# edwinb-ai/MolecularDynamics.jl

Hardware: AMD Instinct MI355X
Metric: particle-steps/sec + achieved HBM GB/s, 1M LJ particles rho=0.897, 1/2/4/8 GPUs (higher is better)
Workload: dtype f64; 1 GPU; BASELINE configs[2]: N=1048576 monodisperse LJ 3D rho=0.897 r_cut=2.5 dt=0.001 NVT Bussi tau=0.1 kT=1.4737, per GPU; particles_per_gpu=1048576, parallelism=1 GPU, step_loop=fused (k_step_tile: one launch per step + k_finalize), global_particles=1048576, tiled_force_kernel=True, max_tile_halo=2081, energies_every_step=False, thermo_frequency=2589

## Files before the change

### include/mdhip.h

```cpp
#ifndef MDHIP_H
#define MDHIP_H

#include <stdint.h>

#ifdef __cplusplus
extern "C" {
#endif

typedef struct md_ctx md_ctx;

enum { MD_POT_LJ = 0, MD_POT_PSEUDOHS = 1, MD_POT_POLYDISPERSE = 2, MD_POT_LJ_MODIFIED = 3, MD_POT_CUSTOM = 100 };

enum { MD_NVE = 0, MD_NVT = 1 };

int md_create(int dim, int64_t n_particles, const double *box, double list_cutoff, int device_id, md_ctx **out);
int md_destroy(md_ctx *ctx);

const char *md_last_error(md_ctx *ctx);

int md_set_potential(md_ctx *ctx, int kind, const double *params, int nparams);

int md_set_potential_source(md_ctx *ctx, const char *hip_src, const char *entry_name, const double *params,
                            int nparams);

// ... 41 lines not shown

int md_stress_setup(md_ctx *ctx, int nlags);
int md_stress_sample(md_ctx *ctx);
int md_stress_tensor(md_ctx *ctx, double *kin, double *vir);
int md_stress_read(md_ctx *ctx, int64_t *nsamples, double *sum_kin, double *sum_vir, int64_t *ncorr, double *corr);
int md_stress_reset(md_ctx *ctx);

int md_kinetic(md_ctx *ctx, double *kinetic);

int md_scale_velocities(md_ctx *ctx, double s);

typedef struct {
    int64_t steps;
    int64_t rebuilds;
    int64_t violations;
    int64_t n_ghost;
    int64_t max_neighbors;
    double avg_neighbors;
    int64_t force_launches;
    double force_ms;
    int64_t max_halo;
    int64_t tiled;
    int64_t prunes;
    int64_t kickdrift_launches;
    double kickdrift_ms;
    int64_t fused;
    int64_t walked_outer;
    int64_t walked_inner;
    int64_t prune_launches_timed;
    double prune_ms;
    int64_t rebuilds_timed;
    double rebuild_ms;
    int64_t fused_build;
} md_stats;
int md_profile(md_ctx *ctx, int enable);
int md_get_stats(md_ctx *ctx, md_stats *out);

int md_create_domain(int dim, int64_t n_global, int64_t n_cap, const double *box, double list_cutoff,
                     int device_id, int rank, int nranks, md_ctx **out);
int md_dom_set_uniform(md_ctx *ctx, int uniform, double sigma);
int md_dom_upload(md_ctx *ctx, int64_t n_own, const int32_t *ids, const double *x, const double *v, const double *f,
                  const int32_t *images, const double *diameters);
int md_dom_download(md_ctx *ctx, int64_t cap, int64_t *n_own, int32_t *ids, double *x, double *v, double *f,
                    int32_t *images);
int md_dom_migrate_pack(md_ctx *ctx, int64_t *nsend );
int md_dom_migrate_unpack(md_ctx *ctx, const int64_t *nrecv );
int md_dom_halo_pack(md_ctx *ctx, int64_t *nsend );
int md_dom_halo_unpack(md_ctx *ctx, const int64_t *nrecv );
int md_dom_build(md_ctx *ctx);
int md_dom_set_step_buffers(md_ctx *ctx, void *send_left, void *send_right, void *recv_left, void *recv_right,
                            int64_t capacity_doubles);
int md_dom_get_sendbuf(md_ctx *ctx, int side, int64_t ndoubles, void *dst, int dst_is_device);
int md_dom_put_recvbuf(md_ctx *ctx, int side, int64_t ndoubles, const void *src, int src_is_device);
int md_dom_step_begin(md_ctx *ctx, double dt, int *violated);
int md_dom_step_end(md_ctx *ctx, double dt, int want_uw, double *uwk);
int md_dom_forces(md_ctx *ctx, double dt, int kick, int want_uw, double *uwk);
int md_dom_set_scale(md_ctx *ctx, double scale);
int md_dom_counts(md_ctx *ctx, int64_t *out );

int md_set_stream(md_ctx *ctx, void *hip_stream);
int md_dom_async_begin(md_ctx *ctx, int64_t nsteps, double dt, int ensemble, double tau, double nf, const double *ktemp,
                       const double *r1, const double *r2, int64_t prune_interval, void *flag_dev ,
                       void *kuw_dev );
int md_dom_step_a(md_ctx *ctx, double dt, int step);
int md_dom_step_b(md_ctx *ctx, double dt, int step, int want_uw);
int md_dom_step_c(md_ctx *ctx, int step, int want_uw);
// ... 19 lines not shown
```

### moleculardynamics/jl_amd/_lib.py

```python
import ctypes as C
import os

_HERE = os.path.dirname(os.path.abspath(__file__))
SO_PATH = os.path.join(_HERE, "csrc", "libmdhip.so")

MD_POT_LJ, MD_POT_PSEUDOHS, MD_POT_POLYDISPERSE, MD_POT_LJ_MODIFIED, MD_POT_CUSTOM = 0, 1, 2, 3, 100
MD_NVE, MD_NVT = 0, 1

EXPORTS = [
    "md_create", "md_destroy", "md_last_error", "md_set_potential", "md_set_potential_source", "md_set_skin",
    "md_set_inner_skin",
    "md_upload", "md_download", "md_snapshot_begin", "md_snapshot_end", "md_compute_forces", "md_neighbor_pairs", "md_run", "md_kinetic",
    "md_scale_velocities", "md_profile", "md_get_stats", "md_version", "md_fire_minimize", "md_run_brownian",
    "md_create_domain", "md_dom_set_uniform", "md_dom_upload", "md_dom_download", "md_dom_migrate_pack",
    "md_dom_migrate_unpack", "md_dom_halo_pack", "md_dom_halo_unpack", "md_dom_build", "md_dom_get_sendbuf",
    "md_dom_put_recvbuf", "md_dom_set_step_buffers", "md_dom_step_begin", "md_dom_step_end", "md_dom_forces", "md_dom_set_scale",
    "md_dom_counts", "md_set_stream", "md_dom_async_begin", "md_dom_step_a", "md_dom_step_b", "md_dom_step_c",
    "md_dom_async_end", "md_dom_comm_unique_id", "md_dom_comm_init", "md_dom_run_window", "md_dom_rebuild",
    "md_dom_enable_pruning", "md_dom_max_disp0", "md_dom_invalidate_inner",
    "md_rdf_setup", "md_rdf_sample", "md_rdf_read", "md_rdf_reset",
    "md_dyn_setup", "md_dyn_origin", "md_dyn_sample", "md_dyn_read", "md_dyn_reset",
    "md_sq_setup", "md_sq_sample", "md_sq_rho", "md_sq_read", "md_sq_reset",
    "md_stress_setup", "md_stress_sample", "md_stress_tensor", "md_stress_read", "md_stress_reset",
]


class MdStats(C.Structure):
    _fields_ = [("steps", C.c_int64), ("rebuilds", C.c_int64), ("violations", C.c_int64), ("n_ghost", C.c_int64),
                ("max_neighbors", C.c_int64), ("avg_neighbors", C.c_double), ("force_launches", C.c_int64),
                ("force_ms", C.c_double), ("max_halo", C.c_int64), ("tiled", C.c_int64), ("prunes", C.c_int64),
                ("kickdrift_launches", C.c_int64), ("kickdrift_ms", C.c_double), ("fused", C.c_int64),
                ("walked_outer", C.c_int64), ("walked_inner", C.c_int64), ("prune_launches_timed", C.c_int64),
                ("prune_ms", C.c_double), ("rebuilds_timed", C.c_int64), ("rebuild_ms", C.c_double),
                ("fused_build", C.c_int64)]


class MdhipError(RuntimeError):
    pass


_lib = None


def load():
    global _lib
    if _lib is not None:
        return _lib
    if not os.path.exists(SO_PATH):
        raise MdhipError(
            f"{SO_PATH} not found: build it with `python -c 'import __graft_entry__ as g; g.build()'` or "
            "`make -C moleculardynamics/jl_amd/csrc`. There is no CPU fallback.")
    L = C.CDLL(SO_PATH)
    vp, dp, ip = C.c_void_p, C.POINTER(C.c_double), C.POINTER(C.c_int32)
    L.md_create.argtypes = [C.c_int, C.c_int64, dp, C.c_double, C.c_int, C.POINTER(vp)]
    L.md_create.restype = C.c_int
    L.md_destroy.argtypes = [vp]
    L.md_destroy.restype = C.c_int
    L.md_last_error.argtypes = [vp]
    L.md_last_error.restype = C.c_char_p
    L.md_set_potential.argtypes = [vp, C.c_int, dp, C.c_int]
    L.md_set_potential.restype = C.c_int
    L.md_set_potential_source.argtypes = [vp, C.c_char_p, C.c_char_p, dp, C.c_int]
    L.md_set_potential_source.restype = C.c_int
    L.md_set_skin.argtypes = [vp, C.c_double]
    L.md_set_skin.restype = C.c_int
    L.md_set_inner_skin.argtypes = [vp, C.c_double]
    L.md_set_inner_skin.restype = C.c_int
# ... 107 lines not shown
```

### moleculardynamics/jl_amd/csrc/md_kernels.hpp

```cpp
#ifndef MD_RTC
#pragma once
#include <hip/hip_runtime.h>
#include <stdint.h>
#else
typedef __hip_internal::uint64_t uint64_t;
typedef __hip_internal::uint32_t uint32_t;
typedef __hip_internal::int32_t int32_t;
typedef __hip_internal::uint16_t uint16_t;
#endif

#define MD_BLOCK 256
#define MD_WAVE 64
#define MD_SENTINEL_POS 1.0e100
#define MD_VAL_SRC_BITS 26
#define MD_VAL_SRC_MASK ((1u << MD_VAL_SRC_BITS) - 1u)
#define MD_NO_VIOLATION 0x7fffffff

enum { POT_LJ = 0, POT_PSEUDOHS = 1, POT_POLYDISPERSE = 2, POT_LJ_MOD = 3, POT_CUSTOM = 100 };

struct DevState {
    double4 *pos;
    double *v[3];
    double *f[3];
    int32_t *img[3];
// ... 823 lines not shown
        uint32_t j = row[(size_t)r * 64];
        uint32_t loc;
        if (j == sentinel) {
            loc = (uint32_t)H;
        } else {
            uint32_t h = (j * 2654435761u) >> (32 - MD_HT_BITS);
            while (keys[h] != j) h = (h + 1) & (MD_HT - 1);
            loc = vals[h];
        }
        row16[row_off(r, lane)] = (uint16_t)(loc * (uint32_t)rs);
    }
}

#ifndef MD_RTC
#include "md_build_tile.hpp"
#endif

struct PruneRow {
    unsigned char *base;
    unsigned off;
};
__device__ __forceinline__ void prune_append(unsigned entry, PruneRow &pr, unsigned long long &acc, int &cin)
{
    unsigned lo = (unsigned)acc, hi = (unsigned)(acc >> 32);
    lo = __builtin_amdgcn_alignbit(hi, lo, 16);
    hi = __builtin_amdgcn_alignbit(entry, hi, 16);
    acc = ((unsigned long long)hi << 32) | lo;
    ++cin;
    if ((cin & 3) == 0) {
        *(unsigned long long *)(pr.base + pr.off) = acc;
        pr.off += 512u;
    }
}

template <int D, int POT, bool UNIFORM, bool WANT_UW, bool PRUNE, int NQ>
__device__ __forceinline__ void tile_pair_block(const unsigned char *smem, const unsigned (&o)[NQ], const double4 &pi,
                                                const PotParams &pp, PruneRow &rin64, double rin2,
                                                unsigned long long &acc, int &cin, double &fx, double &fy, double &fz,
                                                double &us, double &ws, const uint16_t *remap8)
{
    double xj[NQ], yj[NQ], zj[NQ], wj[NQ];
#pragma unroll
    for (int q = 0; q < NQ; ++q) {
        typedef const volatile __attribute__((address_space(3))) double lds_cvd;
        if constexpr (!UNIFORM && D == 3) {
            typedef double md_d2 __attribute__((ext_vector_type(2)));
            typedef const __attribute__((address_space(3))) md_d2 lds_d2;
            lds_d2 *r2 = (lds_d2 *)(smem + o[q]);
            md_d2 a = r2[0], b = r2[1];
            xj[q] = a.x;
            yj[q] = a.y;
            zj[q] = b.x;
            wj[q] = b.y;
        } else {
            lds_cvd *rec = (lds_cvd *)(smem + o[q]);
            xj[q] = rec[0];
            yj[q] = rec[1];
            if constexpr (D == 3) zj[q] = rec[2];
            if constexpr (!UNIFORM) wj[q] = rec[3];
        }
    }
    if constexpr (POT == POT_LJ && UNIFORM && !WANT_UW && D == 3) {
        double dxq[NQ], dyq[NQ], dzq[NQ], dm[NQ];
        unsigned tmin = 0xffffffffu;
        double d2k[PRUNE ? NQ : 1];
#pragma unroll
        for (int q = 0; q < NQ; ++q) {
            dxq[q] = xj[q] - pi.x;
            dyq[q] = yj[q] - pi.y;
            dzq[q] = zj[q] - pi.z;
            double d2 = dxq[q] * dxq[q];
            d2 = __builtin_fma(dyq[q], dyq[q], d2);
            d2 = __builtin_fma(dzq[q], dzq[q], d2);
            if constexpr (PRUNE) d2k[q] = d2;
            int hi = __double2hiint(d2);
            unsigned t = (unsigned)hi - pp.c2_k;
            tmin = min(tmin, t);
            hi = ((int)t < 0) ? hi : 0x5fe00000;
            dm[q] = __hiloint2double(hi, __double2loint(d2));
        }
        if constexpr (PRUNE) {
#pragma unroll
            for (int q = 0; q < NQ; ++q) asm volatile("" : "+v"(d2k[q]));
#pragma unroll
            for (int q = 0; q < NQ; ++q)
                if (d2k[q] <= rin2)
                    prune_append(remap8 ? (unsigned)remap8[o[q] >> 3] : o[q], rin64, acc, cin);
        }
        if (__any(tmin <= 2u)) {
#pragma unroll
            for (int q = 0; q < NQ; ++q) {
                double d2 = dxq[q] * dxq[q];
                d2 = __builtin_fma(dyq[q], dyq[q], d2);
                d2 = __builtin_fma(dzq[q], dzq[q], d2);
                unsigned t = (unsigned)__double2hiint(d2) - pp.c2_k;
                if (t <= 2u) {
                    bool hit = d2_ref<3>(dxq[q], dyq[q], dzq[q]) < pp.c2;
                    dm[q] = __hiloint2double(hit ? __double2hiint(d2) : 0x5fe00000, __double2loint(d2));
                }
            }
        }
#pragma unroll
        for (int q = 0; q < NQ; q += 2) {
            double ip = md_rcp1(dm[q] * dm[q + 1]);
            double z[2] = {dm[q + 1] * ip, dm[q] * ip};
#pragma unroll
            for (int h = 0; h < 2; ++h) {
                double z2 = z[h] * z[h];
                double t = __builtin_fma(pp.ljA, z2 * z[h], -pp.ljB);
                double fpr = (z2 * z2) * t;
                fx = __builtin_fma(-fpr, dxq[q + h], fx);
                fy = __builtin_fma(-fpr, dyq[q + h], fy);
                fz = __builtin_fma(-fpr, dzq[q + h], fz);
            }
        }
    } else
#pragma unroll
    for (int q = 0; q < NQ; ++q) {
        double dx = xj[q] - pi.x;
        double dy = yj[q] - pi.y;
        double dz = 0.0;
        if constexpr (D == 3) dz = zj[q] - pi.z;
        double d2 = d2_ref<D>(dx, dy, dz);
        if constexpr (PRUNE) {
            if (d2 <= rin2)
                prune_append(remap8 ? (unsigned)remap8[o[q] >> 3] : o[q], rin64, acc, cin);
        }
        bool hit = d2 < pp.c2;
        double d2m = mask_d2(d2, hit);
        double u = 0.0, fpr;
        pair_eval<POT, UNIFORM, WANT_UW>(d2m, pi.w, UNIFORM ? 0.0 : wj[q], pp, u, fpr);
        fx = __builtin_fma(-fpr, dx, fx);
        fy = __builtin_fma(-fpr, dy, fy);
        if constexpr (D == 3) fz = __builtin_fma(-fpr, dz, fz);
        if constexpr (WANT_UW) {
            us += u;
            ws = __builtin_fma(fpr, hit ? d2 : 0.0, ws);
        }
    }
}

template <int D, int POT, bool UNIFORM, bool WANT_UW, bool PRUNE>
__device__ __forceinline__ void tile_pair_loop(const unsigned char *smem, const ushort4 *row4,
                                               ushort4 (&jn)[MD_UNROLL / 4], int m_lane, int H,
                                               const double4 &pi, const PotParams &pp, PruneRow &rin64,
                                               double rin2, unsigned long long &acc, int &cin, double &fx, double &fy,
                                               double &fz, double &us, double &ws, const uint16_t *remap8 = nullptr)
{
    constexpr int G = MD_UNROLL / 4;
    static_assert(G == 2, "the tail handling below assumes two groups per iteration");
    (void)H;
    const int m = __builtin_amdgcn_readfirstlane(m_lane);
    int r = 0;
    for (; r + MD_UNROLL <= m; r += MD_UNROLL) {
        unsigned o[MD_UNROLL];
#pragma unroll
        for (int g = 0; g < G; ++g) {
            o[4 * g + 0] = jn[g].x;
            o[4 * g + 1] = jn[g].y;
            o[4 * g + 2] = jn[g].z;
            o[4 * g + 3] = jn[g].w;
        }
#pragma unroll
        for (int g = 0; g < G; ++g) {
            int rg = r + MD_UNROLL + 4 * g;
            jn[g] = row4[(size_t)(((rg < m) ? rg : 0) >> 2) * 64];
        }
        tile_pair_block<D, POT, UNIFORM, WANT_UW, PRUNE, MD_UNROLL>(smem, o, pi, pp, rin64, rin2, acc, cin, fx, fy, fz, us,
                                                                     ws, remap8);
    }
    if (r < m) {
        unsigned o[4] = {jn[0].x, jn[0].y, jn[0].z, jn[0].w};
        tile_pair_block<D, POT, UNIFORM, WANT_UW, PRUNE, 4>(smem, o, pi, pp, rin64, rin2, acc, cin, fx, fy, fz, us, ws,
                                                            remap8);
    }
}

template <int D, bool UNIFORM>
__device__ __forceinline__ void tile_prune_tail(DevState &s, Scalars *sc, int H , int k, bool active, int lane, int wt,
                                                const double4 &pi, PruneRow rin64, int32_t *nmax_in,
                                                unsigned long long acc, int cin)
{
    constexpr int RS = UNIFORM ? 24 : 32;
    {
        const unsigned long long sent = (unsigned long long)(H * RS);
        const unsigned long long sent4 = sent | (sent << 16) | (sent << 32) | (sent << 48);
        int mw = wave_max_i((cin + 3) & ~3);
        int g = cin >> 2;
        if (cin & 3) {
            int p = cin & 3;
            *(unsigned long long *)(rin64.base + rin64.off) = (acc >> (16 * (4 - p))) | (sent4 << (16 * p));
            rin64.off += 512u;
            ++g;
        }
        for (; g < (mw >> 2); ++g, rin64.off += 512u) *(unsigned long long *)(rin64.base + rin64.off) = sent4;
        if (lane == 0) nmax_in[wt] = mw;
        double dd = 0.0;
        if (active) {
#pragma unroll
            for (int c = 0; c < D; ++c) {
                double xc = pos_get(pi, c);
                s.x1[c][k] = xc;
                double d = xc - s.x0[c][k];
                dd = __builtin_fma(d, d, dd);
            }
        }
        double wm = wave_max_d(dd);
// ... 193 lines not shown
                s.v[2][k] = vz;
                ke += vz * vz;
            }
        }
    } else {
        us = 0.0;
        ws = 0.0;
    }
    if constexpr (KICK) {
        double t = block_sum(ke, red);
        if (threadIdx.x == 0) partials[bid] = t;
    }
    if constexpr (WANT_UW) {
        double tu = block_sum(us, red);
        double tw = block_sum(ws, red);
        if (threadIdx.x == 0) {
            partials[nblk_total + bid] = tu;
            partials[2 * nblk_total + bid] = tw;
        }
    }
    MD_SSTAMP(5);
#undef MD_SSTAMP
}

struct StepBufs {
    const double2 *recA;
    double2 *recB;
    size_t rstride;
    const double *fA[3];
    double *fB[3];
    double4 *posB;
};

template <int D, int POT, bool UNIFORM, bool WANT_UW, bool PRUNE>
__global__ void __launch_bounds__(MD_TILE)
    k_step_tile(int n, DevState s, StepBufs sb, PotParams pp, const uint16_t *__restrict__ nlist16, int maxn,
                const int32_t *__restrict__ nmax_tile, const uint32_t *__restrict__ halo, int hcap,
                const int32_t *__restrict__ halo_count, double dt, double skin_half, double inner_half, int use_d1,
                double *__restrict__ partials, int nblk_total, Scalars *__restrict__ sc, int step,
                uint16_t *__restrict__ rows_in, int32_t *__restrict__ nmax_in, double rin2,
                long long *__restrict__ stamps, uint32_t *__restrict__ halo_in, int hcap_in,
                int32_t *__restrict__ halo_in_count, const int32_t *__restrict__ tile_list = nullptr)
{
#define MD_SSTAMP(i)                                                                                   \
    do {                                                                                               \
        if (stamps && (threadIdx.x & 63) == 0)                                                         \
            stamps[((size_t)blockIdx.x * 4 + (threadIdx.x >> 6)) * 8 + (i)] = (long long)clock64();   \
    } while (0)
    constexpr int RS = UNIFORM ? 24 : 32;
    extern __shared__ __attribute__((aligned(16))) unsigned char smem[];
    __shared__ double red[16];
    if (sc->first_viol < step) return;
    MD_SSTAMP(0);
    int bid = xcd_remap(blockIdx.x, gridDim.x);
    if (tile_list) bid = tile_list[bid];
    int H = halo_count[bid];
    const uint32_t *hl = halo + (size_t)bid * hcap;
    int k = bid * MD_TILE + threadIdx.x;
    bool active = k < n;
    int kk = active ? k : n - 1;
    int lane = threadIdx.x & 63;
    int wt = bid * (MD_TILE / 64) + (threadIdx.x >> 6);
    const ushort4 *row4 = (const ushort4 *)(nlist16 + ((size_t)wt * maxn) * 64) + lane;
    PruneRow rin64;
    rin64.base = PRUNE ? (unsigned char *)(rows_in + ((size_t)__builtin_amdgcn_readfirstlane(wt) * maxn) * 64) : nullptr;
    rin64.off = (unsigned)lane * 8u;
    unsigned long long acc = 0ull;
    int cin = 0;
    int m = nmax_tile[wt];
    const double alpha = sc->scale;
    const double adt = alpha * dt;
    const double2 *RA0 = sb.recA, *RA1 = RA0 + sb.rstride, *RA2 = RA1 + sb.rstride, *RA3 = RA2 + sb.rstride;
    double2 a0 = RA0[kk], a1 = RA1[kk], a2 = RA2[kk];
    double sig_own = pp.sig_u;
    if constexpr (!UNIFORM) sig_own = RA3[kk].x;
    double fprev[3] = {0.0, 0.0, 0.0}, xr[3] = {0.0, 0.0, 0.0};
#pragma unroll
    for (int c = 0; c < D; ++c) {
        fprev[c] = sb.fA[c][kk];
        xr[c] = PRUNE ? s.x0[c][kk] : s.x1[c][kk];
    }
    constexpr int G = MD_UNROLL / 4;
    ushort4 jn[G];
#pragma unroll
    for (int g = 0; g < G; ++g) jn[g] = row4[(size_t)((4 * g < m) ? g : 0) * 64];
    MD_SSTAMP(1);
#ifndef MD_STAGE_NB
#define MD_STAGE_NB ((!PRUNE && UNIFORM && !WANT_UW) ? 6 : 8)
#endif
    constexpr int NB = MD_STAGE_NB;
    for (int h0 = 0; h0 <= H; h0 += NB * MD_TILE) {
        uint32_t idx[NB];
#pragma unroll
        for (int i = 0; i < NB; ++i) {
            int h = h0 + i * MD_TILE + threadIdx.x;
            idx[i] = (h < H) ? hl[h] : 0xffffffffu;
        }
        double2 r0[NB], r1[NB], r2[NB], r3[NB];
#pragma unroll
        for (int i = 0; i < NB; ++i) {
            bool ok = idx[i] != 0xffffffffu;
            size_t j = ok ? (size_t)(idx[i] & 0x3ffffffu) : 0;
            r0[i] = RA0[j];
            r1[i] = RA1[j];
            r2[i] = RA2[j];
            if constexpr (!UNIFORM) r3[i] = RA3[j];
        }
#pragma unroll
        for (int i = 0; i < NB; ++i) {
            int h = h0 + i * MD_TILE + threadIdx.x;
            bool ok = idx[i] != 0xffffffffu;
            double x = __builtin_fma(adt, r1[i].y, r0[i].x);
            double y = __builtin_fma(adt, r2[i].x, r0[i].y);
            double z = (D == 3) ? __builtin_fma(adt, r2[i].y, r1[i].x) : 0.0;
            uint32_t code = ok ? (idx[i] >> 26) : 0u;
            if (code) shift_xyz(x, y, z, code, s.boxL, s.tric, s.cellA);
            if (!ok) {
                x = MD_SENTINEL_POS;
                y = MD_SENTINEL_POS;
                z = (D == 3) ? MD_SENTINEL_POS : 0.0;
            }
            if (h <= H) {
                double *rec = (double *)(smem + (size_t)h * RS);
                rec[0] = x;
                rec[1] = y;
                rec[2] = z;
                if constexpr (!UNIFORM) rec[3] = ok ? r3[i].x : 1.0;
            }
        }
    }
    const double pown[3] = {a0.x, a0.y, a1.x}, vown[3] = {a1.y, a2.x, a2.y};
    double vh[3] = {0.0, 0.0, 0.0}, xn[3] = {0.0, 0.0, 0.0};
    double disp2 = 0.0;
#pragma unroll
    for (int c = 0; c < D; ++c) {
        vh[c] = alpha * vown[c] + (fprev[c] * dt) / 2.0;
        xn[c] = __builtin_fma(adt, vown[c], pown[c]);
        double d = xn[c] - xr[c];
        disp2 = __builtin_fma(d, d, disp2);
    }
    const double4 pi = make_double4(xn[0], xn[1], xn[2], sig_own);
    if (active) sb.posB[k] = pi;
    {
        double d1 = use_d1 ? sqrt(__longlong_as_double((long long)sc->d1max2_bits)) : 0.0;
        double thr = fmin(inner_half, skin_half - d1);
        double thr2 = thr > 0.0 ? thr * thr : -1.0;
        if (__any(active && disp2 > thr2)) {
            if (lane == 0) atomicMin(&sc->first_viol, step);
        }
    }
    MD_SSTAMP(2);
    __syncthreads();
    MD_SSTAMP(3);
    double fx = 0.0, fy = 0.0, fz = 0.0, us = 0.0, ws = 0.0;
    tile_pair_loop<D, POT, UNIFORM, WANT_UW, PRUNE>(smem, row4, jn, m, H, pi, pp, rin64, rin2, acc, cin, fx, fy, fz, us, ws, nullptr);
    MD_SSTAMP(4);
    if constexpr (PRUNE) tile_prune_tail<D, UNIFORM>(s, sc, H, k, active, lane, wt, pi, rin64, nmax_in, acc, cin);
    double ke = 0.0;
    if (active) {
        const double fn[3] = {fx, fy, fz};
        const double h2 = (dt * dt) / 2.0;
        double vp[3] = {0.0, 0.0, 0.0}, pn[3] = {0.0, 0.0, 0.0};
#pragma unroll
        for (int c = 0; c < D; ++c) {
            sb.fB[c][k] = fn[c];
            vp[c] = vh[c] + (fn[c] * dt) / 2.0;
            pn[c] = __builtin_fma(h2, fn[c], xn[c]);
            ke += vp[c] * vp[c];
        }
        double2 *RB = sb.recB;
        RB[k] = make_double2(pn[0], pn[1]);
        RB[sb.rstride + k] = make_double2(pn[2], vp[0]);
        RB[2 * sb.rstride + k] = make_double2(vp[1], vp[2]);
        if constexpr (!UNIFORM) RB[3 * sb.rstride + k] = make_double2(sig_own, 0.0);
    } else {
        us = 0.0;
        ws = 0.0;
    }
    {
        double t = block_sum(ke, red);
        if (threadIdx.x == 0) partials[bid] = t;
    }
    if constexpr (WANT_UW) {
        double tu = block_sum(us, red);
        double tw = block_sum(ws, red);
        if (threadIdx.x == 0) {
            partials[nblk_total + bid] = tu;
            partials[2 * nblk_total + bid] = tw;
        }
    }
// ... 468 lines not shown
```

### moleculardynamics/jl_amd/csrc/mdhip.hip

```cpp
#include <cstring>
#include <cstdlib>
#include <unistd.h>

#include "md_kernels.hpp"
#include "md_domain.hpp"
#include "md_rdf.hpp"
#include "md_dyn.hpp"
#include "md_sq.hpp"
#include "md_stress.hpp"

#include <rocprim/rocprim.hpp>

#include <algorithm>
#include <climits>
#include <cmath>
#include <cstdio>
#include <cstring>
#include <stdexcept>
#include <string>
#include <vector>

#include "../../../include/mdhip.h"
#include "md_rtc.hpp"
#include "md_rccl.hpp"
// ... 157 lines not shown
    DBuf<Scalars> scal;
    DBuf<double> d_kt, d_r1, d_r2;

    DBuf<double> io_x, io_v, io_f, io_d;
    DBuf<int32_t> io_i;
    DBuf<double> snap_x;
    DBuf<int32_t> snap_i;
    double *pin_x = nullptr;
    int32_t *pin_i = nullptr;
    size_t pin_n = 0;
    hipStream_t copy_stream = nullptr;
    hipEvent_t ev_snap_ready = nullptr, ev_snap_copied = nullptr;
    bool snap_pending = false;

    bool list_valid = false;
    int64_t steps_since_build = 0;
    int64_t target_interval = 8;
    double inner_skin_req = 0.16;
    double inner_skin = 0.0;
    bool virtual_ghosts = false;
    bool inner_valid = false;
    bool prune_on = false;
    DBuf<double> x1[3];
    DBuf<uint16_t> nlist16_in;
    DBuf<int32_t> nmax_tile_in;
    int64_t steps_since_prune = 0;
    DBuf<double2> rec[2];
    DBuf<uint32_t> halo_in;
    DBuf<int32_t> halo_in_count;
    int hcap_in = 0;
    size_t tile_lds_in = 0;
    bool allow_inner_halo = true;
    bool inner_halo_live = false;
    int fz_a = 0;
    bool allow_fused = true;
    double d1_rate = 0.0;
    bool rate_known = false;
    double safety = 0.97;
    int64_t st_prunes = 0;

    int64_t st_steps = 0, st_rebuilds = 0, st_viol = 0;
    bool prof = false;
    int prof_stride = 1;
    int64_t prof_seen[2] = {0, 0};
    bool prof_open = false;
    std::vector<std::pair<hipEvent_t, hipEvent_t>> prof_ev;
    size_t prof_used = 0;
    double prof_ms_acc = 0.0;
    int64_t prof_launch_acc = 0;
    std::vector<int> prof_tag;
    double prof_kd_ms_acc = 0.0;
    int64_t prof_kd_launch_acc = 0;
    int64_t prof_prune_acc = 0;
    double prof_prune_ms_acc = 0.0;
    double prof_rebuild_ms_acc = 0.0;
    int64_t prof_rebuild_acc = 0;
    bool prof_cur_prune = false;
    bool last_run_fused = false;
    struct StepPart {
        const int32_t *list = nullptr;
        int count = 0;
        hipStream_t stream = nullptr;
        bool last = true;
    } part;

    struct Rdf {
// ... 478 lines not shown
    if (getenv("MDHIP_ROWSTATS")) {
        std::vector<int32_t> nn((size_t)n), nm((size_t)c->ntiles);
        HIPCHK(hipMemcpyAsync(nn.data(), c->nneigh.p, sizeof(int32_t) * n, hipMemcpyDeviceToHost, st));
        HIPCHK(hipMemcpyAsync(nm.data(), c->nmax_tile.p, sizeof(int32_t) * c->ntiles, hipMemcpyDeviceToHost, st));
        HIPCHK(hipStreamSynchronize(st));
        double mean = 0, padded = 0, sorted_p = 0, p8 = 0, s8 = 0;
        for (int i = 0; i < n; ++i) mean += nn[i];
        for (int w = 0; w < (n + 63) / 64; ++w) { padded += nm[w]; p8 += (nm[w] + 7) & ~7; }
        for (int t0 = 0; t0 + 256 <= n; t0 += 256) {
            std::vector<int> v(nn.begin() + t0, nn.begin() + t0 + 256);
            std::sort(v.begin(), v.end());
            for (int w = 0; w < 4; ++w) { int mx = (v[64 * w + 63] + 3) & ~3; sorted_p += mx; s8 += (mx + 7) & ~7; }
        }
        int nw = (n + 63) / 64;
        fprintf(stderr, "[mdhip] rows: mean %.2f  wave-max(4) %.2f  wave-max(8) %.2f  sorted-within-tile(4) %.2f  (8) %.2f\n",
                mean / n, padded / nw, p8 / nw, sorted_p / nw, s8 / nw);
    }
    c->list_valid = true;
    c->steps_since_build = 0;
    c->st_rebuilds++;
    c->inner_valid = false;
    c->prune_on = c->use_tiles && (!c->dom.on || c->dom.prune_enabled) && c->skin > 0.0 && c->inner_skin_req > 0.0 &&
                  c->inner_skin_req < 0.9 * c->skin && c->pot_kind != POT_CUSTOM;
    if (c->prune_on) {
        c->inner_skin = c->inner_skin_req;
        for (int d = 0; d < c->dim; ++d) c->x1[d].ensure(c->ncap);
        c->nlist16_in.ensure((size_t)c->ntiles * c->maxn * 64);
        c->nmax_tile_in.ensure(c->ntiles);
        const size_t target = (c->tile_rs == 24) ? (40 * 1024 - 256) : (53 * 1024);
        int cap_in = (int)std::min<size_t>((size_t)c->hstride, target / c->tile_rs - 1);
        if (c->dom.on || getenv("MDHIP_INNER_CAP_OUTER")) cap_in = c->hstride;
        c->hcap_in = std::max(cap_in, 1);
        c->tile_lds_in = (((size_t)(c->hcap_in + 1) * c->tile_rs) + 15) & ~(size_t)15;
        c->halo_in.ensure((size_t)c->nblk * c->hcap_in);
        c->halo_in_count.ensure(c->nblk);
    }
}

void rebuild(md_ctx *c)
{
    if (c->dim == 3)
        rebuild_t<3>(c);
    else
        rebuild_t<2>(c);
    HIPCHK(hipGetLastError());
}

void prof_begin(md_ctx *c, int tag = 0)
{
    if (!c->prof) return;
    c->prof_open = tag >= 2 || (c->prof_seen[tag]++ % c->prof_stride) == 0;
    if (!c->prof_open) return;
    if (c->prof_used >= c->prof_ev.size()) {
        if (c->prof_ev.size() >= 8192) return;
        hipEvent_t a, b;
        HIPCHK(hipEventCreate(&a));
        HIPCHK(hipEventCreate(&b));
        c->prof_ev.emplace_back(a, b);
        c->prof_tag.push_back(0);
    }
    c->prof_tag[c->prof_used] = tag;
    HIPCHK(hipEventRecord(c->prof_ev[c->prof_used].first, c->stream));
}
void prof_end(md_ctx *c)
{
    if (!c->prof || !c->prof_open) return;
    c->prof_open = false;
    if (c->prof_used >= c->prof_ev.size()) return;
// ... 9 lines not shown
        HIPCHK(hipEventElapsedTime(&ms, c->prof_ev[i].first, c->prof_ev[i].second));
        if (c->prof_tag[i] == 1) {
            c->prof_kd_ms_acc += ms;
            c->prof_kd_launch_acc++;
        } else if (c->prof_tag[i] == 2) {
            c->prof_rebuild_ms_acc += ms;
            c->prof_rebuild_acc++;
        } else if (c->prof_tag[i] == 3) {
            c->prof_prune_ms_acc += ms;
            c->prof_prune_acc++;
        } else {
            c->prof_ms_acc += ms;
            c->prof_launch_acc++;
        }
    }
    c->prof_used = 0;
}

template <int D, int POT, bool UNIFORM>
void launch_force_tpu(md_ctx *c, bool want_uw, bool kick, double dt, int step, int rows)
{
    int n = (int)c->n;
    int nb = c->nblk;
    bool prune_step = rows == 0 && c->prune_on && !c->inner_valid && kick;
    bool use_inner = rows == 0 && c->inner_valid;
    const uint16_t *rows16 = use_inner ? c->nlist16_in.p : c->nlist16.p;
    const int32_t *rowmax = use_inner ? c->nmax_tile_in.p : c->nmax_tile.p;
    const bool ih = c->allow_inner_halo && c->prune_on && c->hcap_in > 0 && c->use_tiles;
    const uint32_t *halo_p = c->halo.p;
    int halo_cap = c->hcap;
    const int32_t *halo_cnt = c->halo_count.p;
    size_t lds_bytes = c->tile_lds;
    uint32_t *hin_p = nullptr;
    if (prune_step && ih) {
        hin_p = c->halo_in.p;
        lds_bytes = ((c->tile_lds + 15) & ~(size_t)15) + (c->tile_lds / 8 + 8) * 2;
        c->inner_halo_live = true;
    } else if (prune_step) {
        c->inner_halo_live = false;
    } else if (use_inner && c->inner_halo_live) {
        halo_p = c->halo_in.p;
        halo_cap = c->hcap_in;
        halo_cnt = c->halo_in_count.p;
        lds_bytes = c->tile_lds_in;
    }
    DevState s = c->dev(c->cur);
    double rin = c->rc + c->inner_skin;
    if (prune_step) {
        for (int d = 0; d < 3; ++d) s.x1[d] = c->x1[d].p;
        k_reset_d1<<<1, 1, 0, c->stream>>>(c->scal.p, step);
    }
#define LF(UW, KK)                                                                                                  \
    k_force<D, POT, UNIFORM, UW, KK><<<nb, MD_BLOCK, 0, c->stream>>>(n, s, c->pp, c->nlist.p, c->maxn,              \
                                                                     c->nmax_tile.p, dt, c->partials.p, nb,         \
                                                                     c->scal.p, step)
#define LT(UW, KK, PR)                                                                                              \
    do {                                                                                                            \
        static int attr_dev_mask = 0;                       \
        auto kfn = k_force_tile<D, POT, UNIFORM, UW, KK, PR>;                                                       \
        if (!(attr_dev_mask & (1 << (c->device & 31)))) {                                                           \
            HIPCHK(hipFuncSetAttribute((const void *)kfn, hipFuncAttributeMaxDynamicSharedMemorySize,               \
                                       (int)(160 * 1024 - 2048)));                                                  \
            attr_dev_mask |= 1 << (c->device & 31);                                                                 \
        }                                                                                                           \
        kfn<<<nb, MD_TILE, lds_bytes, c->stream>>>(n, s, c->pp, rows16, c->maxn, rowmax, halo_p, halo_cap,          \
                                                   halo_cnt, dt, c->partials.p, nb, c->scal.p, step,                \
// ... 231 lines not shown
            k_unfuse<2, true><<<c->nblk, MD_BLOCK, 0, c->stream>>>(n, s, rec, rec_stride(c), c->scal.p, ap);
        else
            k_unfuse<2, false><<<c->nblk, MD_BLOCK, 0, c->stream>>>(n, s, rec, rec_stride(c), c->scal.p, ap);
    }
    c->fz_a = 0;
}

template <int D, int POT, bool UNIFORM>
void launch_step_tpu(md_ctx *c, bool want_uw, double dt, int step)
{
    int n = (int)c->n;
    int nb = c->nblk;
    bool prune_step = c->prune_on && !c->inner_valid;
    bool use_inner = c->inner_valid;
    const uint16_t *rows16 = use_inner ? c->nlist16_in.p : c->nlist16.p;
    const int32_t *rowmax = use_inner ? c->nmax_tile_in.p : c->nmax_tile.p;
    double skin_half = 0.5 * c->skin;
    double inner_half = use_inner ? 0.5 * c->inner_skin : 0.5 * c->skin;
    int use_d1 = use_inner ? 1 : 0;
    DevState s = c->dev(c->cur);
    double rin = c->rc + c->inner_skin;
    const bool whole = c->part.list == nullptr;
    hipStream_t lst = whole ? c->stream : c->part.stream;
    const int grid = whole ? nb : c->part.count;
    if (prune_step) {
        for (int d = 0; d < 3; ++d) s.x1[d] = c->x1[d].p;
        if (whole) k_reset_d1<<<1, 1, 0, c->stream>>>(c->scal.p, step - 1);
    }
    const uint32_t *halo_p = c->halo.p;
    int halo_cap = c->hcap;
    const int32_t *halo_cnt = c->halo_count.p;
    size_t lds_bytes = c->tile_lds;
    uint32_t *hin_p = nullptr;
    if (prune_step) {
        c->inner_halo_live = false;
    } else if (use_inner && c->inner_halo_live) {
        halo_p = c->halo_in.p;
        halo_cap = c->hcap_in;
        halo_cnt = c->halo_in_count.p;
        lds_bytes = c->tile_lds_in;
    }
    const int a = c->fz_a;
    StateBufs &A = c->sb[c->cur ^ a], &B = c->sb[c->cur ^ a ^ 1];
    StepBufs sbufs{};
    sbufs.recA = c->rec[a].p;
    sbufs.recB = c->rec[a ^ 1].p;
    sbufs.rstride = rec_stride(c);
    for (int d = 0; d < 3; ++d) {
        sbufs.fA[d] = A.f[d].p;
        sbufs.fB[d] = B.f[d].p;
    }
    sbufs.posB = B.pos.p;
#define LS(UW, PR)                                                                                                  \
    do {                                                                                                            \
        auto kfn = k_step_tile<D, POT, UNIFORM, UW, PR>;                                                            \
        static int attr_dev_mask = 0;                                                                               \
        if (!(attr_dev_mask & (1 << (c->device & 31)))) {                                                           \
            HIPCHK(hipFuncSetAttribute((const void *)kfn, hipFuncAttributeMaxDynamicSharedMemorySize,               \
                                       (int)(160 * 1024 - 2048)));                                                  \
            attr_dev_mask |= 1 << (c->device & 31);                                                                 \
        }                                                                                                           \
        if (grid > 0)                                                                                               \
            kfn<<<grid, MD_TILE, lds_bytes, lst>>>(n, s, sbufs, c->pp, rows16, c->maxn, rowmax, halo_p, halo_cap,   \
                                                   halo_cnt, dt, skin_half, inner_half, use_d1,                     \
                                                   c->partials.p, nb, c->scal.p, step, c->nlist16_in.p,             \
                                                   c->nmax_tile_in.p, rin * rin, c->dbg_stamps.p, hin_p,            \
                                                   c->hcap_in, c->halo_in_count.p, c->part.list);                   \
    } while (0)
    if (whole) prof_begin(c, prune_step ? 3 : 0);
    if (prune_step) {
        if (want_uw)
            LS(true, true);
        else
            LS(false, true);
    } else {
        if (want_uw)
            LS(true, false);
        else
            LS(false, false);
    }
    if (whole) prof_end(c);
#undef LS
    if (!whole && !c->part.last) return;
    c->fz_a ^= 1;
    if (prune_step) {
        c->inner_valid = true;
        c->steps_since_prune = 0;
        c->st_prunes++;
    }
}

template <int D>
void launch_step_d(md_ctx *c, bool want_uw, double dt, int step)
{
    bool u = c->uniform_sigma;
    switch (c->pot_kind) {
    case POT_LJ:
        if (u)
            launch_step_tpu<D, POT_LJ, true>(c, want_uw, dt, step);
        else
// ... 186 lines not shown
            HIPCHK(hipDeviceGetStreamPriorityRange(&plo, &phi));
            HIPCHK(hipStreamCreateWithPriority(&ctx->stream, hipStreamNonBlocking, phi));
        } else {
            HIPCHK(hipStreamCreateWithFlags(&ctx->stream, hipStreamNonBlocking));
        }
        ctx->own_stream = ctx->stream;
        ctx->dim = dim;
        ctx->n_global = n_global;
        ctx->ncap = n_cap;
        ctx->n = domain ? 0 : n_cap;
        for (int c = 0; c < dim; ++c) ctx->L[c] = box[c * dim + c];
        ctx->tric = cg.tric;
        for (int c = 0; c < 9; ++c) {
            ctx->A[c] = cg.A[c];
            ctx->Ainv[c] = cg.Ainv[c];
        }
        for (int c = 0; c < 3; ++c) ctx->perp[c] = cg.perp[c];
        ctx->volume = cg.volume;
        ctx->rc = list_cutoff;
        if (domain) {
            ctx->dom.on = true;
            ctx->skin_req = 0.4;
            ctx->dom.rank = rank;
            ctx->dom.nranks = nranks;
            ctx->dom.xlo = ctx->L[0] * rank / nranks;
            ctx->dom.xhi = (rank == nranks - 1) ? ctx->L[0] : ctx->L[0] * (rank + 1) / nranks;
        }
        if (const char *e = getenv("MDHIP_NO_TILES")) ctx->allow_tiles = !(e[0] == '1');
        if (const char *e = getenv("MDHIP_NO_FUSED_BUILD")) ctx->allow_fused_build = !(e[0] == '1');
        if (const char *e = getenv("MDHIP_INNER_SKIN")) ctx->inner_skin_req = atof(e);
        if (const char *e = getenv("MDHIP_NO_FUSED_STEP")) ctx->allow_fused = !(e[0] == '1');
        ctx->allow_inner_halo = false;
        if (const char *e = getenv("MDHIP_INNER_HALO")) ctx->allow_inner_halo = (e[0] == '1');
        ctx->pot_kind = POT_LJ;
        ctx->pp.p[0] = 1.0;
        ctx->pp.p[1] = 1.0;
        ctx->pp.p[2] = 2.5;
        configure_grid(ctx);
        configure_potential(ctx);
        double frac = 1.0;
        for (int c = 0; c < dim; ++c) frac *= (double)ctx->grid.ncx[c] / ctx->grid.nc[c];
        int64_t gcap = (int64_t)((frac - 1.0) * 1.3 * n_cap) + 4096;
        ctx->cap = n_cap + gcap;
        alloc_state(ctx, 0, ctx->cap);
        alloc_state(ctx, 1, ctx->cap);
        int64_t n = n_cap;
        ctx->nimg.alloc(ctx->cap + 2);
        ctx->img_off.alloc(ctx->cap + 2);
        HIPCHK(hipMemsetAsync(ctx->nimg.p, 0, sizeof(int32_t) * (ctx->cap + 2), ctx->stream));
        ctx->newslot.alloc(ctx->cap + 1);
        ctx->keys_in.alloc(ctx->cap);
        ctx->keys_out.alloc(ctx->cap);
        ctx->vals_in.alloc(ctx->cap);
        ctx->vals_out.alloc(ctx->cap);
        ctx->gsrc.alloc(ctx->cap + 1);
        ctx->gcode.alloc(ctx->cap + 1);
        ctx->gowner.alloc(ctx->cap + 1);
        ctx->nblk = nblocks(ctx->n);
        int nblk_cap = nblocks(n);
        ctx->ntiles = (int64_t)nblk_cap * (MD_BLOCK / 64);
        ctx->nneigh.alloc(n);
        ctx->nmax_tile.alloc(ctx->ntiles);
        double dens = (double)n_global;
        dens /= ctx->volume;
        double vol = (dim == 3) ? 4.18879020478639 * ctx->rl * ctx->rl * ctx->rl : 3.14159265358979 * ctx->rl * ctx->rl;
        int maxn = (int)(dens * vol * 1.35) + 24;
// ... 1431 lines not shown
        std::vector<int32_t> h((size_t)ctx->n);
        HIPCHK(hipMemcpyAsync(h.data(), ctx->nneigh.p, sizeof(int32_t) * ctx->n, hipMemcpyDeviceToHost, ctx->stream));
        HIPCHK(hipStreamSynchronize(ctx->stream));
        double sum = 0.0;
        for (int32_t v : h) sum += v;
        out->avg_neighbors = sum / (double)ctx->n;
    }
    out->prunes = ctx->st_prunes;
    out->max_halo = ctx->use_tiles ? ctx->hstride : 0;
    out->tiled = ctx->use_tiles ? 1 : 0;
    out->force_launches = ctx->prof_launch_acc;
    out->force_ms = ctx->prof_ms_acc;
    out->kickdrift_launches = ctx->prof_kd_launch_acc;
    out->kickdrift_ms = ctx->prof_kd_ms_acc;
    out->fused = ctx->last_run_fused ? 1 : 0;
    out->walked_outer = out->walked_inner = 0;
    if (ctx->list_valid) {
        const int64_t nw = (ctx->n + 63) / 64;
        std::vector<int32_t> h((size_t)nw);
        HIPCHK(hipMemcpyAsync(h.data(), ctx->nmax_tile.p, sizeof(int32_t) * nw, hipMemcpyDeviceToHost, ctx->stream));
        HIPCHK(hipStreamSynchronize(ctx->stream));
        for (int32_t v : h) out->walked_outer += 64 * (int64_t)v;
        if (ctx->inner_valid) {
            HIPCHK(hipMemcpyAsync(h.data(), ctx->nmax_tile_in.p, sizeof(int32_t) * nw, hipMemcpyDeviceToHost, ctx->stream));
            HIPCHK(hipStreamSynchronize(ctx->stream));
            for (int32_t v : h) out->walked_inner += 64 * (int64_t)v;
        }
    }
    out->prune_launches_timed = ctx->prof_prune_acc;
    out->prune_ms = ctx->prof_prune_ms_acc;
    out->rebuilds_timed = ctx->prof_rebuild_acc;
    out->rebuild_ms = ctx->prof_rebuild_ms_acc;
    out->fused_build = (ctx->list_valid && ctx->use_tiles && !ctx->have_nlist32) ? 1 : 0;
    API_END
}


namespace {
void dom_require(md_ctx *c)
{
    if (!c->dom.on) throw HipError("this handle was not created with md_create_domain");
}
DomCounters dom_read_counters(md_ctx *c)
{
    DomCounters h;
    HIPCHK(hipMemcpyAsync(&h, c->dom.counters.p, sizeof h, hipMemcpyDeviceToHost, c->stream));
    HIPCHK(hipStreamSynchronize(c->stream));
    if (h.error & 1) throw HipError("a particle moved by more than one slab between list builds");
    if (h.error & 2) throw HipError("slab exchange buffer overflow (raise n_cap)");
    return h;
}
}

int md_dom_set_uniform(md_ctx *ctx, int uniform, double sigma)
{
    API_BEGIN
    dom_require(ctx);
    ctx->uniform_sigma = uniform != 0;
    ctx->sigma_u = sigma;
    configure_potential(ctx);
    ctx->list_valid = false;
    API_END
}

int md_dom_upload(md_ctx *ctx, int64_t n_own, const int32_t *ids, const double *x, const double *v, const double *f,
                  const int32_t *images, const double *diameters)
// ... 1312 lines not shown
```

Baseline: 6.689 billion particle-steps/s.

## Stage only inner-list-referenced halo particles on non-prune fused steps

During prune steps, the fused step kernel now marks in shared memory which halo slots fall inside the inner cutoff. It then emits a compacted per-tile list of those halo entries, plus owned particles, together with their original LDS slot indices. Later non-prune steps stage only these entries into shared memory instead of the whole halo, which cuts gather traffic. The cost is atomics and an extra scan on prune steps, sentinel handling for slots left unstaged, and a change of the staging batch size for the uniform non-energy case.

Result: no change. 6.631 billion particle-steps/s (-0.9%).

```diff
diff --git a/include/mdhip.h b/include/mdhip.h
--- a/include/mdhip.h
+++ b/include/mdhip.h
@@ -97,6 +97,9 @@
     int64_t rebuilds_timed;
     double rebuild_ms;
     int64_t fused_build;
+    double staged_inner;
+    double staged_outer;
+    int64_t staged_over;
 } md_stats;
 int md_profile(md_ctx *ctx, int enable);
 int md_get_stats(md_ctx *ctx, md_stats *out);
diff --git a/moleculardynamics/jl_amd/_lib.py b/moleculardynamics/jl_amd/_lib.py
--- a/moleculardynamics/jl_amd/_lib.py
+++ b/moleculardynamics/jl_amd/_lib.py
@@ -32,7 +32,8 @@
                 ("kickdrift_launches", C.c_int64), ("kickdrift_ms", C.c_double), ("fused", C.c_int64),
                 ("walked_outer", C.c_int64), ("walked_inner", C.c_int64), ("prune_launches_timed", C.c_int64),
                 ("prune_ms", C.c_double), ("rebuilds_timed", C.c_int64), ("rebuild_ms", C.c_double),
-                ("fused_build", C.c_int64)]
+                ("fused_build", C.c_int64), ("staged_inner", C.c_double), ("staged_outer", C.c_double),
+                ("staged_over", C.c_int64)]
 
 
 class MdhipError(RuntimeError):
diff --git a/moleculardynamics/jl_amd/csrc/md_kernels.hpp b/moleculardynamics/jl_amd/csrc/md_kernels.hpp
--- a/moleculardynamics/jl_amd/csrc/md_kernels.hpp
+++ b/moleculardynamics/jl_amd/csrc/md_kernels.hpp
@@ -879,12 +879,18 @@
         pr.off += 512u;
     }
 }
-
-template <int D, int POT, bool UNIFORM, bool WANT_UW, bool PRUNE, int NQ>
+template <bool MARK>
+__device__ __forceinline__ void prune_mark(unsigned *marks, unsigned o)
+{
+    if constexpr (MARK)
+        __hip_atomic_fetch_or(marks + (o >> 8), 1u << ((o >> 3) & 31u), __ATOMIC_RELAXED, __HIP_MEMORY_SCOPE_WORKGROUP);
+}
+
+template <int D, int POT, bool UNIFORM, bool WANT_UW, bool PRUNE, int NQ, bool MARK = false>
 __device__ __forceinline__ void tile_pair_block(const unsigned char *smem, const unsigned (&o)[NQ], const double4 &pi,
                                                 const PotParams &pp, PruneRow &rin64, double rin2,
                                                 unsigned long long &acc, int &cin, double &fx, double &fy, double &fz,
-                                                double &us, double &ws, const uint16_t *remap8)
+                                                double &us, double &ws, const uint16_t *remap8, unsigned *marks = nullptr)
 {
     double xj[NQ], yj[NQ], zj[NQ], wj[NQ];
 #pragma unroll
@@ -931,8 +937,10 @@
             for (int q = 0; q < NQ; ++q) asm volatile("" : "+v"(d2k[q]));
 #pragma unroll
             for (int q = 0; q < NQ; ++q)
-                if (d2k[q] <= rin2)
+                if (d2k[q] <= rin2) {
                     prune_append(remap8 ? (unsigned)remap8[o[q] >> 3] : o[q], rin64, acc, cin);
+                    prune_mark<MARK>(marks, o[q]);
+                }
         }
         if (__any(tmin <= 2u)) {
 #pragma unroll
@@ -970,8 +978,10 @@
         if constexpr (D == 3) dz = zj[q] - pi.z;
         double d2 = d2_ref<D>(dx, dy, dz);
         if constexpr (PRUNE) {
-            if (d2 <= rin2)
+            if (d2 <= rin2) {
                 prune_append(remap8 ? (unsigned)remap8[o[q] >> 3] : o[q], rin64, acc, cin);
+                prune_mark<MARK>(marks, o[q]);
+            }
         }
         bool hit = d2 < pp.c2;
         double d2m = mask_d2(d2, hit);
@@ -987,12 +997,13 @@
     }
 }
 
-template <int D, int POT, bool UNIFORM, bool WANT_UW, bool PRUNE>
+template <int D, int POT, bool UNIFORM, bool WANT_UW, bool PRUNE, bool MARK = false>
 __device__ __forceinline__ void tile_pair_loop(const unsigned char *smem, const ushort4 *row4,
                                                ushort4 (&jn)[MD_UNROLL / 4], int m_lane, int H,
                                                const double4 &pi, const PotParams &pp, PruneRow &rin64,
                                                double rin2, unsigned long long &acc, int &cin, double &fx, double &fy,
-                                               double &fz, double &us, double &ws, const uint16_t *remap8 = nullptr)
+                                               double &fz, double &us, double &ws, const uint16_t *remap8 = nullptr,
+                                               unsigned *marks = nullptr)
 {
     constexpr int G = MD_UNROLL / 4;
     static_assert(G == 2, "the tail handling below assumes two groups per iteration");
@@ -1013,13 +1024,13 @@
             int rg = r + MD_UNROLL + 4 * g;
             jn[g] = row4[(size_t)(((rg < m) ? rg : 0) >> 2) * 64];
         }
-        tile_pair_block<D, POT, UNIFORM, WANT_UW, PRUNE, MD_UNROLL>(smem, o, pi, pp, rin64, rin2, acc, cin, fx, fy, fz, us,
-                                                                     ws, remap8);
+        tile_pair_block<D, POT, UNIFORM, WANT_UW, PRUNE, MD_UNROLL, MARK>(smem, o, pi, pp, rin64, rin2, acc, cin, fx, fy, fz,
+                                                                           us, ws, remap8, marks);
     }
     if (r < m) {
         unsigned o[4] = {jn[0].x, jn[0].y, jn[0].z, jn[0].w};
-        tile_pair_block<D, POT, UNIFORM, WANT_UW, PRUNE, 4>(smem, o, pi, pp, rin64, rin2, acc, cin, fx, fy, fz, us, ws,
-                                                            remap8);
+        tile_pair_block<D, POT, UNIFORM, WANT_UW, PRUNE, 4, MARK>(smem, o, pi, pp, rin64, rin2, acc, cin, fx, fy, fz, us, ws,
+                                                                  remap8, marks);
     }
 }
 
@@ -1279,6 +1290,131 @@
     double4 *posB;
 };
 
+template <bool UNIFORM>
+__device__ __forceinline__ void tile_sparse_emit(const unsigned *marks, int H, const uint32_t *hl, int bid,
+                                                 uint32_t *__restrict__ halo_in, uint16_t *__restrict__ slot_in, int hcap,
+                                                 int32_t *__restrict__ halo_in_count)
+{
+    constexpr unsigned RS8 = UNIFORM ? 3u : 4u;
+    __shared__ int sh_scan3[16];
+    __syncthreads();
+    const uint32_t own0 = (uint32_t)bid * MD_TILE;
+    uint32_t *lo = halo_in + (size_t)bid * hcap;
+    uint16_t *so = slot_in + (size_t)bid * hcap;
+    int carry = 0;
+    for (int h0 = 0; h0 < H; h0 += 8 * MD_TILE) {
+        const int hb = h0 + 8 * (int)threadIdx.x;
+        uint32_t e[8];
+        unsigned keep = 0u;
+#pragma unroll
+        for (int i = 0; i < 8; ++i) {
+            int h = hb + i;
+            e[i] = (h < H) ? hl[h] : 0u;
+            if (h < H) {
+                unsigned b = (unsigned)h * RS8;
+                bool marked = (marks[b >> 5] >> (b & 31u)) & 1u;
+                bool own = (e[i] >> 26) == 0u && (e[i] - own0) < (uint32_t)MD_TILE;
+                if (marked || own) keep |= 1u << i;
+            }
+        }
+        int tot;
+        int base = carry + block_excl_scan(__popc(keep), sh_scan3, &tot);
+#pragma unroll
+        for (int i = 0; i < 8; ++i) {
+            if ((keep >> i) & 1u) {
+                if (base < hcap) {
+                    lo[base] = e[i];
+                    so[base] = (uint16_t)(hb + i);
+                }
+                ++base;
+            }
+        }
+        carry += tot;
+    }
+    if (threadIdx.x == 0) halo_in_count[bid] = carry;
+}
+
+template <int D, bool UNIFORM, int NB, bool FULL, bool SPARSE>
+__device__ __forceinline__ void stage_batch(unsigned char *smem, const DevState &s, const double2 *RA0, size_t rstride,
+                                            const uint32_t *lst, const uint16_t *sl, int j0, int nst, int Hs, double adt)
+{
+    constexpr int RS = UNIFORM ? 24 : 32;
+    const char *B0 = (const char *)RA0, *B1 = B0 + rstride * sizeof(double2), *B2 = B1 + rstride * sizeof(double2),
+               *B3 = B2 + rstride * sizeof(double2);
+    uint32_t idx[NB];
+    unsigned slot[NB];
+#pragma unroll
+    for (int i = 0; i < NB; ++i) {
+        const int j = j0 + i * MD_TILE + (int)threadIdx.x;
+        if constexpr (FULL) {
+            idx[i] = lst[j];
+            slot[i] = SPARSE ? (unsigned)sl[j] : (unsigned)j;
+        } else {
+            idx[i] = 0xffffffffu;
+            slot[i] = (unsigned)Hs;
+            if (j0 + i * MD_TILE <= nst) {
+                if (j < nst) {
+                    idx[i] = lst[j];
+                    slot[i] = SPARSE ? (unsigned)sl[j] : (unsigned)j;
+                }
+            }
+        }
+    }
+    double2 r0[NB], r1[NB], r2[NB], r3[NB];
+#pragma unroll
+    for (int i = 0; i < NB; ++i) {
+        if (FULL || j0 + i * MD_TILE <= nst) {
+            uint32_t src = idx[i] & 0x3ffffffu;
+            if constexpr (!FULL) src = (idx[i] != 0xffffffffu) ? src : 0u;
+            const uint32_t off = src << 4;
+            r0[i] = *(const double2 *)(B0 + off);
+            r1[i] = *(const double2 *)(B1 + off);
+            r2[i] = *(const double2 *)(B2 + off);
+            if constexpr (!UNIFORM) r3[i] = *(const double2 *)(B3 + off);
+        }
+    }
+#pragma unroll
+    for (int i = 0; i < NB; ++i) {
+        if (FULL || j0 + i * MD_TILE <= nst) {
+            const int j = j0 + i * MD_TILE + (int)threadIdx.x;
+            double x = __builtin_fma(adt, r1[i].y, r0[i].x);
+            double y = __builtin_fma(adt, r2[i].x, r0[i].y);
+            double z = (D == 3) ? __builtin_fma(adt, r2[i].y, r1[i].x) : 0.0;
+            double w = UNIFORM ? 0.0 : r3[i].x;
+            uint32_t code = idx[i] >> 26;
+            if constexpr (!FULL) {
+                if (idx[i] == 0xffffffffu) code = 0u;
+            }
+            if (code) shift_xyz(x, y, z, code, s.boxL, s.tric, s.cellA);
+            if constexpr (!FULL) {
+                if (idx[i] == 0xffffffffu) {
+                    x = MD_SENTINEL_POS;
+                    y = MD_SENTINEL_POS;
+                    z = (D == 3) ? MD_SENTINEL_POS : 0.0;
+                    w = 1.0;
+                }
+            }
+            if (FULL || j <= nst) {
+                double *rec = (double *)(smem + slot[i] * (unsigned)RS);
+                rec[0] = x;
+                rec[1] = y;
+                rec[2] = z;
+                if constexpr (!UNIFORM) rec[3] = w;
+            }
+        }
+    }
+}
+
+template <int D, bool UNIFORM, int NB, bool SPARSE>
+__device__ __forceinline__ void stage_list(unsigned char *smem, const DevState &s, const double2 *RA0, size_t rstride,
+                                           const uint32_t *lst, const uint16_t *sl, int nst, int Hs, double adt)
+{
+    int j0 = 0;
+    for (; j0 + NB * MD_TILE <= nst; j0 += NB * MD_TILE)
+        stage_batch<D, UNIFORM, NB, true, SPARSE>(smem, s, RA0, rstride, lst, sl, j0, nst, Hs, adt);
+    stage_batch<D, UNIFORM, NB, false, SPARSE>(smem, s, RA0, rstride, lst, sl, j0, nst, Hs, adt);
+}
+
 template <int D, int POT, bool UNIFORM, bool WANT_UW, bool PRUNE>
 __global__ void __launch_bounds__(MD_TILE)
     k_step_tile(int n, DevState s, StepBufs sb, PotParams pp, const uint16_t *__restrict__ nlist16, int maxn,
@@ -1287,7 +1423,8 @@
                 double *__restrict__ partials, int nblk_total, Scalars *__restrict__ sc, int step,
                 uint16_t *__restrict__ rows_in, int32_t *__restrict__ nmax_in, double rin2,
                 long long *__restrict__ stamps, uint32_t *__restrict__ halo_in, int hcap_in,
-                int32_t *__restrict__ halo_in_count, const int32_t *__restrict__ tile_list = nullptr)
+                int32_t *__restrict__ halo_in_count, const int32_t *__restrict__ tile_list = nullptr,
+                uint16_t *__restrict__ slot_in = nullptr)
 {
 #define MD_SSTAMP(i)                                                                                   \
     do {                                                                                               \
@@ -1333,49 +1470,22 @@
     for (int g = 0; g < G; ++g) jn[g] = row4[(size_t)((4 * g < m) ? g : 0) * 64];
     MD_SSTAMP(1);
 #ifndef MD_STAGE_NB
-#define MD_STAGE_NB ((!PRUNE && UNIFORM && !WANT_UW) ? 6 : 8)
+#define MD_STAGE_NB ((!PRUNE && UNIFORM && !WANT_UW) ? 4 : 8)
 #endif
     constexpr int NB = MD_STAGE_NB;
-    for (int h0 = 0; h0 <= H; h0 += NB * MD_TILE) {
-        uint32_t idx[NB];
-#pragma unroll
-        for (int i = 0; i < NB; ++i) {
-            int h = h0 + i * MD_TILE + threadIdx.x;
-            idx[i] = (h < H) ? hl[h] : 0xffffffffu;
-        }
-        double2 r0[NB], r1[NB], r2[NB], r3[NB];
-#pragma unroll
-        for (int i = 0; i < NB; ++i) {
-            bool ok = idx[i] != 0xffffffffu;
-            size_t j = ok ? (size_t)(idx[i] & 0x3ffffffu) : 0;
-            r0[i] = RA0[j];
-            r1[i] = RA1[j];
-            r2[i] = RA2[j];
-            if constexpr (!UNIFORM) r3[i] = RA3[j];
-        }
-#pragma unroll
-        for (int i = 0; i < NB; ++i) {
-            int h = h0 + i * MD_TILE + threadIdx.x;
-            bool ok = idx[i] != 0xffffffffu;
-            double x = __builtin_fma(adt, r1[i].y, r0[i].x);
-            double y = __builtin_fma(adt, r2[i].x, r0[i].y);
-            double z = (D == 3) ? __builtin_fma(adt, r2[i].y, r1[i].x) : 0.0;
-            uint32_t code = ok ? (idx[i] >> 26) : 0u;
-            if (code) shift_xyz(x, y, z, code, s.boxL, s.tric, s.cellA);
-            if (!ok) {
-                x = MD_SENTINEL_POS;
-                y = MD_SENTINEL_POS;
-                z = (D == 3) ? MD_SENTINEL_POS : 0.0;
-            }
-            if (h <= H) {
-                double *rec = (double *)(smem + (size_t)h * RS);
-                rec[0] = x;
-                rec[1] = y;
-                rec[2] = z;
-                if constexpr (!UNIFORM) rec[3] = ok ? r3[i].x : 1.0;
-            }
-        }
-    }
+    unsigned *marks = nullptr;
+    if constexpr (PRUNE) {
+        if (slot_in) {
+            marks = (unsigned *)(smem + ((((size_t)(H + 1) * RS) + 15) & ~(size_t)15));
+            const int nw = ((((H + 1) * RS) >> 3) + 32) >> 5;
+            for (int w = threadIdx.x; w < nw; w += MD_TILE) marks[w] = 0u;
+        }
+    }
+    if (!PRUNE && slot_in)
+        stage_list<D, UNIFORM, NB, true>(smem, s, RA0, sb.rstride, halo_in + (size_t)bid * hcap_in,
+                                         slot_in + (size_t)bid * hcap_in, halo_in_count[bid], H, adt);
+    else
+        stage_list<D, UNIFORM, NB, false>(smem, s, RA0, sb.rstride, hl, nullptr, H, H, adt);
     const double pown[3] = {a0.x, a0.y, a1.x}, vown[3] = {a1.y, a2.x, a2.y};
     double vh[3] = {0.0, 0.0, 0.0}, xn[3] = {0.0, 0.0, 0.0};
     double disp2 = 0.0;
@@ -1400,9 +1510,17 @@
     __syncthreads();
     MD_SSTAMP(3);
     double fx = 0.0, fy = 0.0, fz = 0.0, us = 0.0, ws = 0.0;
-    tile_pair_loop<D, POT, UNIFORM, WANT_UW, PRUNE>(smem, row4, jn, m, H, pi, pp, rin64, rin2, acc, cin, fx, fy, fz, us, ws, nullptr);
+    if (PRUNE && marks)
+        tile_pair_loop<D, POT, UNIFORM, WANT_UW, PRUNE, PRUNE>(smem, row4, jn, m, H, pi, pp, rin64, rin2, acc, cin, fx, fy, fz,
+                                                               us, ws, nullptr, marks);
+    else
+        tile_pair_loop<D, POT, UNIFORM, WANT_UW, PRUNE>(smem, row4, jn, m, H, pi, pp, rin64, rin2, acc, cin, fx, fy, fz, us, ws,
+                                                        nullptr);
     MD_SSTAMP(4);
-    if constexpr (PRUNE) tile_prune_tail<D, UNIFORM>(s, sc, H, k, active, lane, wt, pi, rin64, nmax_in, acc, cin);
+    if constexpr (PRUNE) {
+        tile_prune_tail<D, UNIFORM>(s, sc, H, k, active, lane, wt, pi, rin64, nmax_in, acc, cin);
+        if (marks) tile_sparse_emit<UNIFORM>(marks, H, hl, bid, halo_in, slot_in, hcap_in, halo_in_count);
+    }
     double ke = 0.0;
     if (active) {
         const double fn[3] = {fx, fy, fz};
diff --git a/moleculardynamics/jl_amd/csrc/mdhip.hip b/moleculardynamics/jl_amd/csrc/mdhip.hip
--- a/moleculardynamics/jl_amd/csrc/mdhip.hip
+++ b/moleculardynamics/jl_amd/csrc/mdhip.hip
@@ -213,6 +213,10 @@
     size_t tile_lds_in = 0;
     bool allow_inner_halo = true;
     bool inner_halo_live = false;
+    DBuf<uint16_t> slot_in;
+    bool allow_sparse_stage = true;
+    bool sparse_live = false;
+    bool last_ord_sparse = false;
     int fz_a = 0;
     bool allow_fused = true;
     double d1_rate = 0.0;
@@ -757,8 +761,9 @@
         if (c->dom.on || getenv("MDHIP_INNER_CAP_OUTER")) cap_in = c->hstride;
         c->hcap_in = std::max(cap_in, 1);
         c->tile_lds_in = (((size_t)(c->hcap_in + 1) * c->tile_rs) + 15) & ~(size_t)15;
-        c->halo_in.ensure((size_t)c->nblk * c->hcap_in);
+        c->halo_in.ensure((size_t)c->nblk * std::max(c->hcap_in, c->hcap));
         c->halo_in_count.ensure(c->nblk);
+        c->slot_in.ensure((size_t)c->nblk * c->hcap);
     }
 }
 
@@ -834,6 +839,7 @@
     const int32_t *halo_cnt = c->halo_count.p;
     size_t lds_bytes = c->tile_lds;
     uint32_t *hin_p = nullptr;
+    if (prune_step) c->sparse_live = false;
     if (prune_step && ih) {
         hin_p = c->halo_in.p;
         lds_bytes = ((c->tile_lds + 15) & ~(size_t)15) + (c->tile_lds / 8 + 8) * 2;
@@ -1131,14 +1137,28 @@
     const int32_t *halo_cnt = c->halo_count.p;
     size_t lds_bytes = c->tile_lds;
     uint32_t *hin_p = nullptr;
+    uint16_t *slot_p = nullptr;
+    int hin_cap = c->hcap_in;
     if (prune_step) {
         c->inner_halo_live = false;
+        c->sparse_live = c->allow_sparse_stage;
+        if (c->sparse_live) {
+            hin_p = c->halo_in.p;
+            slot_p = c->slot_in.p;
+            hin_cap = c->hcap;
+            lds_bytes = ((c->tile_lds + 15) & ~(size_t)15) + c->tile_lds / 64 + 16;
+        }
     } else if (use_inner && c->inner_halo_live) {
         halo_p = c->halo_in.p;
         halo_cap = c->hcap_in;
         halo_cnt = c->halo_in_count.p;
         lds_bytes = c->tile_lds_in;
-    }
+    } else if (use_inner && c->sparse_live) {
+        hin_p = c->halo_in.p;
+        slot_p = c->slot_in.p;
+        hin_cap = c->hcap;
+    }
+    if (!prune_step && (whole || c->part.last)) c->last_ord_sparse = slot_p != nullptr;
     const int a = c->fz_a;
     StateBufs &A = c->sb[c->cur ^ a], &B = c->sb[c->cur ^ a ^ 1];
     StepBufs sbufs{};
@@ -1164,7 +1184,7 @@
                                                    halo_cnt, dt, skin_half, inner_half, use_d1,                     \
                                                    c->partials.p, nb, c->scal.p, step, c->nlist16_in.p,             \
                                                    c->nmax_tile_in.p, rin * rin, c->dbg_stamps.p, hin_p,            \
-                                                   c->hcap_in, c->halo_in_count.p, c->part.list);                   \
+                                                   hin_cap, c->halo_in_count.p, c->part.list, slot_p);              \
     } while (0)
     if (whole) prof_begin(c, prune_step ? 3 : 0);
     if (prune_step) {
@@ -1417,6 +1437,7 @@
         if (const char *e = getenv("MDHIP_NO_FUSED_STEP")) ctx->allow_fused = !(e[0] == '1');
         ctx->allow_inner_halo = false;
         if (const char *e = getenv("MDHIP_INNER_HALO")) ctx->allow_inner_halo = (e[0] == '1');
+        if (const char *e = getenv("MDHIP_SPARSE_STAGE")) ctx->allow_sparse_stage = !(e[0] == '0');
         ctx->pot_kind = POT_LJ;
         ctx->pp.p[0] = 1.0;
         ctx->pp.p[1] = 1.0;
@@ -2914,6 +2935,25 @@
     out->rebuilds_timed = ctx->prof_rebuild_acc;
     out->rebuild_ms = ctx->prof_rebuild_ms_acc;
     out->fused_build = (ctx->list_valid && ctx->use_tiles && !ctx->have_nlist32) ? 1 : 0;
+    out->staged_inner = out->staged_outer = 0.0;
+    out->staged_over = 0;
+    if (ctx->list_valid && ctx->use_tiles && ctx->nblk > 0) {
+        const size_t nb = (size_t)ctx->nblk;
+        std::vector<int32_t> ho(nb), hi(nb);
+        HIPCHK(hipMemcpyAsync(ho.data(), ctx->halo_count.p, sizeof(int32_t) * nb, hipMemcpyDeviceToHost, ctx->stream));
+        const bool sparse = ctx->inner_valid && ctx->sparse_live && ctx->last_ord_sparse && ctx->halo_in_count.n >= nb;
+        if (sparse)
+            HIPCHK(hipMemcpyAsync(hi.data(), ctx->halo_in_count.p, sizeof(int32_t) * nb, hipMemcpyDeviceToHost, ctx->stream));
+        HIPCHK(hipStreamSynchronize(ctx->stream));
+        double so = 0.0, si = 0.0;
+        for (size_t b = 0; b < nb; ++b) {
+            so += ho[b];
+            si += sparse ? hi[b] : ho[b];
+            if (sparse && hi[b] > ho[b]) out->staged_over++;
+        }
+        out->staged_outer = so / (double)nb;
+        out->staged_inner = si / (double)nb;
+    }
     API_END
 }
 
```
